# liayan/Legion-1

Measured on AMD Instinct MI355X. Metric: sampled edges/s + feature GB/s, 3-hop GraphSAGE ogbn-papers100M at 1/2/4/8 GPU, higher is better.
Workload: dtype int32 ids / f32 rows (verbatim copy)

## Files before the change

legion-1_amd/csrc/internal.h:

```cpp
#pragma once
#include <hip/hip_runtime.h>
#include <cstdint>
#include <cstdio>
#include <cstdlib>
#include <iostream>
#include <string>
#include <vector>

#include "../../include/legion_amd.h"
#include "audit.h"

namespace legion {

void report_error(const char* file, int line, const char* msg, bool hip_failure);
bool error_pending();
bool error_is_fatal();
int64_t ipc_max_bytes();
bool ipc_size_ok(int64_t bytes, const char* who);
bool ipc_export_ok(const void* ptr, const char* who);
int64_t shard_chunk_bytes();
inline void check(hipError_t e, const char* file, int line)
{
    if (e != hipSuccess) report_error(file, line, hipGetErrorString(e), true);
}
#define HIP_CHECK(expr) ::legion::check((expr), __FILE__, __LINE__)
#define HIP_CHECK_LAST() ::legion::check(hipGetLastError(), __FILE__, __LINE__)
#define LEGION_ARG_ERROR(msg) ::legion::report_error(__FILE__, __LINE__, (msg), false)

std::ostream& log_out();
FILE* log_file();

int physical_device(int logical);
bool is_remote_device(int logical);
struct DeviceGuard {
    int prev = -1, prev_logical = -1;
    explicit DeviceGuard(int logical);
    ~DeviceGuard();
};

int chunk_shift(int64_t unit_bytes, int min_shift);
inline int chunk_count(int64_t n, int shift) { return n > 0 ? (int)(((n - 1) >> shift) + 1) : 1; }
template <typename T>
struct ChunkList {
    std::vector<T*> chunks;
    bool imported = false;
    T* at(int q) const { return q >= 0 && q < (int)chunks.size() ? chunks[q] : nullptr; }
    bool complete(size_t n) const { for (T* p : chunks) if (!p) return false; return chunks.size() == n; }
    void release();
    int export_chunk(int dev, int q, void* handle64, const char* who) const;
    int import_chunk(int q, const void* handle64, int64_t floor_bytes, int open_dev, const char* who);
};
template <typename T> void upload_table(int viewer, const std::vector<T*>& h, T**& tab, bool realloc, const char* what);

typedef unsigned long long pos_t;
constexpr int kPosShift = 32;
constexpr uint32_t kProvisional = 0x80000000u, kPosValueMask = 0x7FFFFFFFu;
constexpr uint32_t kEpochTop = 0xFFFFFFFFu, kSerialLimit = 0xFFFFFFF0u;
__host__ __device__ inline pos_t pos_entry(uint32_t epoch, uint32_t value) { return ((pos_t)epoch << kPosShift) | (pos_t)value; }
#ifndef LEGION_KTILE
#define LEGION_KTILE 1024
#endif
constexpr int kTile = LEGION_KTILE;
constexpr int kBlock = 256;
static_assert(kTile >= kBlock && kTile <= 2048 && (kTile & (kTile - 1)) == 0, "LEGION_KTILE: a power of two in [256, 2048] (k_sample stages 16 bytes of row descriptor per slot in static LDS)");
constexpr int kMaxChunks = 2048;
static_assert(kMaxChunks % kBlock == 0 && kMaxChunks >= 256 * 8, "kMaxChunks: a multiple of the workgroup size, >= 256 CUs x 8 workgroups");
constexpr int ilog2_c(int v) { return v <= 1 ? 0 : 1 + ilog2_c(v >> 1); }
constexpr int kMaxParts = LEGION_MAX_DEVICE;

constexpr int kModes = 3;
static_assert(LEGION_TRAINMODE == 0 && LEGION_VALIDMODE == 1 && LEGION_TESTMODE == 2, "seed sets are indexed by mode");
struct BuildInfoSeedFields {
    const int32_t* LegionBuildInfo::*num;
    const int32_t* const* LegionBuildInfo::*ids;
    const int32_t* const* LegionBuildInfo::*labels;
};
constexpr BuildInfoSeedFields kBuildInfoSeeds[kModes] = {
    {&LegionBuildInfo::training_set_num, &LegionBuildInfo::training_set_ids, &LegionBuildInfo::training_labels},
    {&LegionBuildInfo::validation_set_num, &LegionBuildInfo::validation_set_ids, &LegionBuildInfo::validation_labels},
    {&LegionBuildInfo::testing_set_num, &LegionBuildInfo::testing_set_ids, &LegionBuildInfo::testing_labels}};

constexpr uint32_t kP31 = 2147483647u;
constexpr uint32_t kA = 48271u;

__host__ __device__ inline uint32_t mulmod31(uint32_t a, uint32_t b)
{
    uint64_t p = (uint64_t)a * (uint64_t)b;
    uint32_t r = (uint32_t)(p & kP31) + (uint32_t)(p >> 31);
    r = (r & kP31) + (r >> 31);
    return r >= kP31 ? r - kP31 : r;
}

__host__ __device__ inline uint32_t powmod31(uint32_t base, uint64_t e)
{
    uint32_t r = 1;
    while (e) {
        if (e & 1) r = mulmod31(r, base);
        base = mulmod31(base, base);
        e >>= 1;
    }
    return r;
}

struct FastDiv {
    uint32_t d = 1, m = 0, s = 0;
    FastDiv() = default;
    explicit FastDiv(uint32_t div);
};

struct CsrTables {
    const int64_t* indptr;
    const int32_t* indices;
    const int64_t* const* frag_indptr;
    const int32_t* const* frag_indices;
    int32_t ip_nch, ix_nch, row_shift, edge_shift;
    int32_t partition_count;
    const int8_t* topo_owner;
// ... 223 lines not shown
```

legion-1_amd/csrc/kernels.hip:

```cpp
#include "internal.h"
#include <hipcub/hipcub.hpp>
#include <mutex>
#include <cstring>

#include "audit_hooks.h"

namespace legion {

__device__ inline int32_t sample_index(uint32_t x, int32_t deg)
{
    double result = (double)(uint32_t)(x - 1u);
    result /= 2147483646.0;
    return (int32_t)(result * (double)deg + 0.0);
}

__device__ inline uint32_t fdiv(uint32_t n, const FastDiv& d)
{
    return d.d == 1 ? n : (uint32_t)(((uint64_t)n * d.m) >> d.s);
}

__device__ inline int lane_id() { return threadIdx.x & 63; }
__device__ inline int wave_id() { return threadIdx.x >> 6; }

__device__ inline int32_t total_nodes(const int32_t* nc, int32_t hops) { return nc[5 + 2 * hops]; }
// ... 45 lines not shown
    const int64_t n_init = min((int64_t)max(size, 0) * f_next, (int64_t)aux_cap);
    for (int64_t i = idx; i < n_init; i += (int64_t)gridDim.x * blockDim.x) aux_next[i] = -1;
}
__global__ void k_fill_aux(const int32_t* __restrict__ nc, int32_t count, int32_t* __restrict__ aux, int32_t aux_cap)
{
    const int64_t n = min((int64_t)nc[2] * count, (int64_t)aux_cap);
    for (int64_t i = threadIdx.x + (int64_t)blockDim.x * blockIdx.x; i < n; i += (int64_t)gridDim.x * blockDim.x) aux[i] = -1;
}
__global__ void k_set_cursor(BatchCtl* ctl, int32_t counter, uint32_t epoch) { ctl->counter = counter; ctl->epoch = epoch; }
__global__ void k_advance(BatchCtl* ctl) { ctl->counter += 1; ctl->epoch -= 1; }


struct SampleArgs {
    CsrTables csr;
    const int32_t* sampled_ids;
    const int32_t* agg_src_ids;
    const int32_t* nc;
    const int32_t* ec;
    pos_t* pos_map;
    int32_t* cand;
    int32_t* aux;
    int32_t* tile_edge;
    unsigned long long* edge_access_time;
    const BatchCtl* ctl;
    const uint32_t* pow_tab;
    uint32_t a_tile;
    uint32_t a_step;
    FastDiv fdiv;
    int32_t count;
    int32_t op_id;
    int32_t window;
    int32_t prefilter_from_op;
};

__device__ inline int32_t claim_slot(const SampleArgs& a, uint32_t epoch, int32_t dst, int32_t idx)
{
    const pos_t prov0 = pos_entry(epoch, kProvisional);
    const pos_t mine = prov0 | (pos_t)(uint32_t)idx;
    pos_t cur = (a.op_id < a.prefilter_from_op) ? ~(pos_t)0 : a.pos_map[dst];
    if (cur > mine) {
        const pos_t old = atomicMin(a.pos_map + dst, mine);
        if (old > mine) {
            if ((uint32_t)(old >> kPosShift) == epoch) a.aux[(uint32_t)old & kPosValueMask] = -2 - idx;
            cur = mine;
        } else {
            cur = old;
        }
    }
    if (cur < prov0) return (int32_t)((uint32_t)cur & kPosValueMask);
    if (cur < mine) return -2 - (int32_t)((uint32_t)cur & kPosValueMask);
    return -1;
}

template <bool PRESC, bool PARTITIONED>
__global__ __launch_bounds__(kBlock) void k_sample(SampleArgs a)
{
    __shared__ const int32_t* s_row[kTile + 2];
    __shared__ int32_t s_deg[kTile + 2];
    __shared__ int32_t s_src[kTile + 2];
    __shared__ int32_t s_cnt[kBlock / 64];

    const int32_t N = a.nc[2];
    const int32_t f = a.count;
    const int32_t total = N * f;
    const int32_t* __restrict__ input = (a.op_id == 2) ? a.sampled_ids : a.agg_src_ids + a.ec[2];
    const int32_t n_tiles = (total + kTile - 1) / kTile;
    const int tid = threadIdx.x;
    const uint32_t epoch = a.ctl->epoch;

    if ((int32_t)blockIdx.x >= n_tiles) return;

    uint32_t x[kTile / kBlock];
    {
        uint32_t base = powmod31(a.a_tile, (uint64_t)blockIdx.x);
#pragma unroll
        for (int s = 0; s < kTile / kBlock; s++) x[s] = mulmod31(base, a.pow_tab[tid + kBlock * s]);
    }

    for (int32_t tile = blockIdx.x; tile < n_tiles; tile += gridDim.x) {
        const int32_t tile_start = tile * kTile;
        const int32_t tile_end = min(tile_start + kTile, total);
        const int32_t i0 = (int32_t)fdiv((uint32_t)tile_start, a.fdiv);
        const int32_t i_last = (int32_t)fdiv((uint32_t)(tile_end - 1), a.fdiv);
        const int32_t nrows = i_last - i0 + 1;

        for (int32_t r = tid; r < nrows; r += kBlock) {
            const int32_t src = input[i0 + r];
            const int32_t* rowp = nullptr;
            int32_t deg = -1;
            if (src >= 0) {
                const int64_t* ip = a.csr.indptr + src;
                const int32_t* ix = a.csr.indices;
                int8_t owner = -1;
                if (PARTITIONED && !PRESC) owner = a.csr.topo_owner[src];
                if (owner >= 0) {
                    const int32_t row = a.csr.topo_row[src];
                    ip = a.csr.frag_indptr[owner * a.csr.ip_nch + (row >> a.csr.row_shift)] + (row & ((1 << a.csr.row_shift) - 1));
                    const int64_t start = ip[0];
                    ix = a.csr.frag_indices[owner * a.csr.ix_nch + (int32_t)(start >> a.csr.edge_shift)];
                    rowp = ix + (start & ((1ll << a.csr.edge_shift) - 1));
                    deg = (int32_t)(ip[1] - start);
                } else {
                    const int64_t start = ip[0];
                    rowp = ix + start;
                    deg = (int32_t)(ip[1] - start);
                }
            }
            s_row[r] = rowp;
            s_deg[r] = deg;
            s_src[r] = src;
        }
        __syncthreads();

        int32_t cnt = 0;
#pragma unroll
        for (int s = 0; s < kTile / kBlock; s++) {
            const int32_t idx = tile_start + tid + kBlock * s;
            int32_t dst = -1, known = -1, j = 0, r = 0;
            if (idx < tile_end) {
                const uint32_t i = fdiv((uint32_t)idx, a.fdiv);
                j = idx - (int32_t)i * f;
                r = (int32_t)i - i0;
                const int32_t deg = s_deg[r];
                if (j < deg) {
                    dst = s_row[r][sample_index(x[s], deg)];
                    if (dst < 0) dst = -1;
                }
            }
            int32_t dup = 0;
            for (int d = 1; d <= a.window; d++) {
                const int32_t o = __shfl_up(dst, d);
                if (d <= j && d <= lane_id() && o == dst) dup = d;
            }
            if (dst >= 0) {
                if (PRESC) atomicAdd(a.edge_access_time + s_src[r], 1ull);
                if (dup) known = -2 - (idx - dup);
                else known = claim_slot(a, epoch, dst, idx);
                cnt++;
            }
            if (idx < tile_end) {
                a.cand[idx] = dst;
                if (dst < 0) a.aux[idx] = 0;
                else if (known != -1) a.aux[idx] = known;
            }
        }
        for (int o = 32; o > 0; o >>= 1) cnt += __shfl_down(cnt, o);
        if (lane_id() == 0) s_cnt[wave_id()] = cnt;
        __syncthreads();
        if (tid == 0) {
            int32_t t = 0;
#pragma unroll
            for (int w = 0; w < kBlock / 64; w++) t += s_cnt[w];
            a.tile_edge[tile] = t;
        }
#pragma unroll
        for (int s = 0; s < kTile / kBlock; s++) x[s] = mulmod31(x[s], a.a_step);
        __syncthreads();
    }
}

constexpr int32_t kWinBase = 0x40000000;

__device__ inline int32_t enc_win(int32_t r) { return -2 - (kWinBase + r); }
__device__ inline bool is_win(int32_t v) { return v <= -2 - kWinBase; }
__device__ inline int32_t win_rank(int32_t v) { return -2 - v - kWinBase; }

__host__ __device__ inline FastDiv make_fastdiv(uint32_t div)
{
    FastDiv f;
    f.d = div ? div : 1;
    if (f.d == 1) { f.m = 0; f.s = 0; return f; }
    uint32_t l = 0;
    while ((1ull << l) < f.d) l++;
    f.m = (uint32_t)(((1ull << (31 + l)) / f.d) + 1ull);
    f.s = 31 + l;
    return f;
}

__global__ __launch_bounds__(kBlock) void k_mark(const int32_t* __restrict__ nc, const int32_t* __restrict__ ec,
                                                 int32_t count, int32_t* __restrict__ aux, const int32_t* __restrict__ tile_edge,
                                                 int32_t* __restrict__ tile_node, int2* __restrict__ tile_pre,
                                                 int2* __restrict__ chunk_tot, HopState* __restrict__ hs)
{
    constexpr int S = kTile / kBlock, W = kBlock / 64;
    __shared__ int32_t s_c[S * W];
    const int32_t total = nc[2] * count;
    const int32_t n_tiles = (total + kTile - 1) / kTile;
    const int lane = lane_id(), wave = wave_id();
    const unsigned long long lt = (1ull << lane) - 1ull;
    if (blockIdx.x == 0 && threadIdx.x == 0) {
        HopState h;
        h.edge_base = ec[0]; h.node_base = nc[0]; h.n_edges = 0; h.n_nodes = 0;
        h.in_off = ec[2]; h.n_in = nc[2]; h.slots = total; h.pad = 0;
        *hs = h;
    }
    const int32_t T = (n_tiles + (int32_t)gridDim.x - 1) / (int32_t)gridDim.x;
    const int32_t t0 = (int32_t)blockIdx.x * T, t1 = min(t0 + T, n_tiles);
    if (t0 >= n_tiles) return;
    int32_t nxt[S];
#pragma unroll
    for (int s = 0; s < S; s++) {
        const int64_t idx = (int64_t)t0 * kTile + threadIdx.x + kBlock * s;
        nxt[s] = idx < total ? aux[idx] : 0;
    }
    int32_t te_next = threadIdx.x == 0 ? tile_edge[t0] : 0, run_e = 0, run_n = 0;
    for (int32_t tile = t0; tile < t1; tile++) {
        bool win[S];
        int32_t rk[S];
        const int32_t te = te_next;
#pragma unroll
        for (int s = 0; s < S; s++) {
            const int32_t idx = tile * kTile + threadIdx.x + kBlock * s;
            win[s] = idx < total && nxt[s] == -1;
        }
        {
            const int64_t nt = (int64_t)tile + 1;
#pragma unroll
            for (int s = 0; s < S; s++) {
                const int64_t idx = nt * kTile + threadIdx.x + kBlock * s;
                nxt[s] = (nt < t1 && idx < total) ? aux[idx] : 0;
            }
            if (threadIdx.x == 0 && nt < t1) te_next = tile_edge[nt];
        }
#pragma unroll
        for (int s = 0; s < S; s++) {
            const unsigned long long b = __ballot(win[s]);
            rk[s] = __popcll(b & lt);
            if (lane == 0) s_c[s * W + wave] = __popcll(b);
        }
        __syncthreads();
        int32_t run = 0, before[S];
#pragma unroll
        for (int q = 0; q < S * W; q++) {
#pragma unroll
            for (int s = 0; s < S; s++)
                if (q == s * W + wave) before[s] = run;
            run += s_c[q];
        }
#pragma unroll
        for (int s = 0; s < S; s++)
            if (win[s]) aux[tile * kTile + threadIdx.x + kBlock * s] = enc_win(before[s] + rk[s]);
        if (threadIdx.x == 0) {
            tile_node[tile] = run;
            tile_pre[tile] = make_int2(run_e, run_n);
            run_e += te; run_n += run;
        }
        __syncthreads();
    }
    if (threadIdx.x == 0) chunk_tot[blockIdx.x] = make_int2(run_e, run_n);
}

__device__ inline void apply_update_counter(int32_t* nc, int32_t* ec, int32_t op_id, int32_t hops, int32_t n_nodes,
                                            int32_t n_edges)
{
    const int32_t hh = op_id / 2;
    nc[0] += n_nodes;
    nc[3 + 2 * hh] = nc[1 + 2 * hh] + nc[2 + 2 * hh];
    nc[4 + 2 * hh] = n_nodes;
    if (hh == hops) nc[5 + 2 * hh] = nc[3 + 2 * hh] + nc[4 + 2 * hh];
    nc[1] = 0;
    nc[2] = n_edges;
    ec[2 + hh] = (hh == 1 ? ec[3] : ec[1 + hh]) + n_edges;
    ec[2] = ec[0];
    ec[0] += n_edges;
    ec[1] = 0;
}

struct WriteArgs {
    HopState* hs;
    int32_t* nc;
    int32_t* ec;
    int32_t hops;
    const int32_t* cand;
    const int32_t* aux;
    const int32_t* tile_edge;
    const int32_t* tile_node;
    int32_t* sampled_ids;
    int32_t* agg_src_ids;
    int32_t* agg_src_off;
    int32_t* agg_dst_off;
    pos_t* pos_map;
    FastDiv fdiv;
    int32_t op_id;
    const BatchCtl* ctl;
    int32_t last_hop;
    const int2* tile_pre;
    const int2* chunk_tot;
    int32_t mark_grid;
    int32_t* aux_next;
    int32_t next_count;
    int32_t aux_cap;
    int32_t ids_cap;
    int32_t V;
};

#define LEGION_STORE_OK(i, cap) ((uint32_t)(i) < (uint32_t)(cap))

__global__ __launch_bounds__(kBlock) void k_write(WriteArgs a)
{
    constexpr int S = kTile / kBlock, W = kBlock / 64;
    __shared__ int2 s_chunk[kMaxChunks];
    __shared__ int32_t s_e[S * W];
    __shared__ int2 s_scan[W];
    __shared__ uint32_t s_div_t[3];
    const HopState h = *a.hs;
    const uint32_t epoch = a.ctl->epoch;
    const int32_t total = h.slots;
    const int32_t n_tiles = (total + kTile - 1) / kTile;
    const int lane = lane_id(), wave = wave_id();
    const unsigned long long lt = (1ull << lane) - 1ull;
    if (n_tiles == 0) {
        if (blockIdx.x == 0 && threadIdx.x == 0) apply_update_counter(a.nc, a.ec, a.op_id, a.hops, 0, 0);
        return;
    }
    if ((int32_t)blockIdx.x >= n_tiles) return;
    const int32_t T = (n_tiles + a.mark_grid - 1) / a.mark_grid;
    if (threadIdx.x == 0) {
        const FastDiv f = make_fastdiv((uint32_t)T);
        s_div_t[0] = f.d; s_div_t[1] = f.m; s_div_t[2] = f.s;
    }
    const int32_t n_chunks = (n_tiles + T - 1) / T;
    {
        constexpr int PER = kMaxChunks / kBlock;
        const int32_t q0 = (int32_t)threadIdx.x * PER;
        int2 v[PER];
#pragma unroll
        for (int u = 0; u < PER; u++) v[u] = a.chunk_tot[min(q0 + u, n_chunks - 1)];
        int32_t se = 0, sn = 0;
#pragma unroll
        for (int u = 0; u < PER; u++) {
            if (q0 + u >= n_chunks) v[u] = make_int2(0, 0);
            se += v[u].x; sn += v[u].y;
        }
        int32_t ie = se, in = sn;
        for (int o = 1; o < 64; o <<= 1) {
            const int32_t ue = __shfl_up(ie, o), un = __shfl_up(in, o);
            if (lane >= o) { ie += ue; in += un; }
        }
        if (lane == 63) s_scan[wave] = make_int2(ie, in);
        __syncthreads();
        int32_t run_e = ie - se, run_n = in - sn;
#pragma unroll
        for (int w = 0; w < W; w++)
            if (w < wave) { run_e += s_scan[w].x; run_n += s_scan[w].y; }
#pragma unroll
        for (int u = 0; u < PER; u++) {
            if (q0 + u < n_chunks) s_chunk[q0 + u] = make_int2(run_e, run_n);
            run_e += v[u].x; run_n += v[u].y;
        }
        __syncthreads();
    }
    FastDiv div_t;
    div_t.d = s_div_t[0]; div_t.m = s_div_t[1]; div_t.s = s_div_t[2];
    auto nodes_before = [&](int32_t t, int32_t pre_n_in_chunk) { return s_chunk[fdiv((uint32_t)t, div_t)].y + pre_n_in_chunk; };

    for (int32_t tile = blockIdx.x; tile < n_tiles; tile += gridDim.x) {
        const int2 own = a.tile_pre[tile], own_chunk = s_chunk[fdiv((uint32_t)tile, div_t)];
        const int32_t pre_e = own_chunk.x + own.x, pre_n = own_chunk.y + own.y;
        const int32_t tile_e = a.tile_edge[tile];
        const int32_t ebase = h.edge_base + pre_e;
        const int32_t nbase = h.node_base + pre_n;
        int32_t c[S], so[S], dpos[S], w[S], re[S], wpre[S];
        const int32_t* __restrict__ pre_n_of = reinterpret_cast<const int32_t*>(a.tile_pre) + 1;
#pragma unroll
        for (int s = 0; s < S; s++) {
            const int32_t idx = tile * kTile + threadIdx.x + kBlock * s;
            c[s] = (idx < total) ? a.cand[idx] : -1;
            so[s] = (idx < total) ? a.aux[idx] : 0;
        }
#pragma unroll
        for (int s = 0; s < S; s++) {
            dpos[s] = 0; w[s] = -1;
            if (c[s] == -1) continue;
            const int32_t idx = tile * kTile + threadIdx.x + kBlock * s;
            const int32_t i = (int32_t)fdiv((uint32_t)idx, a.fdiv);
            dpos[s] = (a.op_id == 2) ? (int32_t)((uint32_t)a.pos_map[a.sampled_ids[i]] & kPosValueMask) : a.agg_src_off[h.in_off + i];
            wpre[s] = 0;
            if (so[s] < -1 && !is_win(so[s])) { w[s] = -2 - so[s]; so[s] = a.aux[w[s]]; wpre[s] = pre_n_of[2 * (w[s] / kTile)]; }
        }
#pragma unroll
        for (int s = 0; s < S; s++)
            while (w[s] >= 0 && so[s] < -1 && !is_win(so[s])) { w[s] = -2 - so[s]; so[s] = a.aux[w[s]]; wpre[s] = pre_n_of[2 * (w[s] / kTile)]; }
#pragma unroll
        for (int s = 0; s < S; s++) {
            const unsigned long long be = __ballot(c[s] != -1);
            re[s] = __popcll(be & lt);
            if (lane == 0) s_e[s * W + wave] = __popcll(be);
        }
        __syncthreads();
        if (tile == n_tiles - 1 && threadIdx.x == 0) {
            const int32_t n_edges = pre_e + tile_e, n_nodes = pre_n + a.tile_node[tile];
            a.hs->n_edges = n_edges;
            a.hs->n_nodes = n_nodes;
            apply_update_counter(a.nc, a.ec, a.op_id, a.hops, n_nodes, n_edges);
        }
#pragma unroll
        for (int s = 0; s < S; s++) {
            if (c[s] == -1) continue;
            int32_t pe = 0;
            for (int q = 0; q < s * W + wave; q++) pe += s_e[q];
            const int32_t dst = c[s];
            const int32_t e = ebase + pe + re[s];
            if (!LEGION_STORE_OK(e, a.ids_cap)) continue;
            if (!a.last_hop) a.agg_src_ids[e] = dst;
            a.agg_dst_off[e] = dpos[s];
            int32_t p = so[s];
            if (w[s] >= 0) {
                if (p < -1)
                    p = h.node_base + nodes_before(w[s] / kTile, wpre[s]) + win_rank(p);
            } else if (is_win(p)) {
                p = nbase + win_rank(p);
                if (LEGION_STORE_OK(p, a.ids_cap)) a.sampled_ids[p] = dst;
                if (!a.last_hop && LEGION_STORE_OK(dst, a.V)) a.pos_map[dst] = pos_entry(epoch, (uint32_t)p);
            }
            a.agg_src_off[e] = p;
        }
        if (a.next_count > 0) {
            const int64_t lo = min((int64_t)pre_e * a.next_count, (int64_t)a.aux_cap);
            const int64_t hi = min((int64_t)(pre_e + tile_e) * a.next_count, (int64_t)a.aux_cap);
            for (int64_t q = lo + threadIdx.x; q < hi; q += kBlock) a.aux_next[q] = -1;
        }
        __syncthreads();
    }
}

__global__ __launch_bounds__(kBlock) void k_find_feat(const int32_t* __restrict__ sampled_ids,
                                                      int32_t* __restrict__ cache_offset,
                                                      const int32_t* __restrict__ nc, int32_t off_idx,
                                                      int32_t size_idx, const int32_t* __restrict__ feat_map)
{
    const int32_t off = nc[off_idx], n = nc[size_idx];
    for (int32_t r = threadIdx.x + blockDim.x * blockIdx.x; r < n; r += gridDim.x * blockDim.x) {
        int32_t id = sampled_ids[off + r];
        cache_offset[r] = (id < 0 || !feat_map) ? -1 : feat_map[id];
    }
}

__global__ __launch_bounds__(kBlock) void k_find_topo(const int32_t* __restrict__ input_ids,
                                                      int8_t* __restrict__ part_index,
                                                      int32_t* __restrict__ part_offset, int32_t n,
                                                      const int8_t* __restrict__ owner,
                                                      const int32_t* __restrict__ row)
{
    for (int32_t i = threadIdx.x + blockDim.x * blockIdx.x; i < n; i += gridDim.x * blockDim.x) {
        int32_t id = input_ids[i];
        bool ok = id >= 0 && owner;
        part_index[i] = ok ? owner[id] : (int8_t)-1;
        part_offset[i] = ok ? row[id] : -1;
    }
}

struct GatherKArgs {
    GatherArgs g;
    FastDiv div_c;
    FastDiv div_cap;
};

typedef float v4f __attribute__((ext_vector_type(4)));

__global__ __launch_bounds__(kBlock) void k_row_ptrs(GatherKArgs a)
{
    constexpr int U = 4;
// ... 389 lines not shown
}
static inline int grid_for(int64_t work_items, int per_block, int blocks_per_cu = 8)
{
    int64_t need = (work_items + per_block - 1) / per_block;
    int64_t cap = (int64_t)cu_count() * blocks_per_cu;
    if (need < 1) need = 1;
    return (int)(need < cap ? need : cap);
}

static uint32_t* pow_table()
{
    static uint32_t* tabs[64] = {nullptr};
    static std::mutex mu;
    std::lock_guard<std::mutex> lk(mu);
    int dev = 0;
    HIP_CHECK(hipGetDevice(&dev));
    if (!tabs[dev]) {
        std::vector<uint32_t> h(kTile);
        uint32_t x = 1;
        for (int m = 0; m < kTile; m++) { x = mulmod31(x, kA); h[m] = x; }
        HIP_CHECK(hipMalloc(&tabs[dev], kTile * sizeof(uint32_t)));
        HIP_CHECK(hipMemcpy(tabs[dev], h.data(), kTile * sizeof(uint32_t), hipMemcpyHostToDevice));
    }
    LEGION_AUDIT_SHARE(tabs[dev], current_logical_device());
    return tabs[dev];
}

void launch_seed(hipStream_t s, int32_t* batch_ids, int32_t* labels, int32_t batch_size, int32_t size, int32_t counter,
                 const int32_t* all_ids, const int32_t* all_labels, int32_t total_cap, pos_t* pos_map,
                 uint32_t epoch, BatchCtl* ctl, bool self_driven, int32_t* nc, int32_t* ec, int32_t* aux_next,
                 int32_t f_next, int32_t aux_cap)
{
    const int32_t bound = self_driven ? batch_size : size;
    int blocks = bound > 0 ? (bound - 1) / kBlock + 1 : 1;
    LEGION_AUDIT_LAUNCH(s, "k_seed", LEGION_AW(batch_ids), LEGION_AW(labels), LEGION_AW(pos_map), LEGION_AW(ctl), LEGION_AW(nc), LEGION_AW(ec), LEGION_AW(aux_next), LEGION_AL(all_ids), LEGION_AL(all_labels));
    if (self_driven) k_seed<true><<<blocks, kBlock, 0, s>>>(batch_ids, labels, batch_size, size, counter, all_ids, all_labels, total_cap, pos_map, epoch, ctl, nc, ec, aux_next, f_next, aux_cap);
    else k_seed<false><<<blocks, kBlock, 0, s>>>(batch_ids, labels, batch_size, size, counter, all_ids, all_labels, total_cap, pos_map, epoch, ctl, nc, ec, aux_next, f_next, aux_cap);
    HIP_CHECK_LAST();
}
void launch_set_cursor(hipStream_t s, BatchCtl* ctl, int32_t counter, uint32_t epoch)
{
    LEGION_AUDIT_LAUNCH(s, "k_set_cursor", LEGION_AW(ctl));
    k_set_cursor<<<1, 1, 0, s>>>(ctl, counter, epoch);
    HIP_CHECK_LAST();
}
void launch_advance(hipStream_t s, BatchCtl* ctl)
{
    LEGION_AUDIT_LAUNCH(s, "k_advance", LEGION_AW(ctl));
    k_advance<<<1, 1, 0, s>>>(ctl);
    HIP_CHECK_LAST();
}
void warm_static_tables() { (void)pow_table(); (void)cu_count(); }

void launch_sample_hop(hipStream_t s, const CsrTables& csr, const SamplerBuffers& b, int32_t count, int32_t op_id,
                       int32_t hops, int32_t slots_bound, bool is_presc)
{
    if (count <= 0 || slots_bound <= 0) { LEGION_ARG_ERROR("GPU_Random_Sampling: empty hop"); return; }
    const int max_tiles = (slots_bound + kTile - 1) / kTile;
    constexpr int wg_per_cu = 4;
    const int grid = std::min(grid_for(max_tiles, 1, wg_per_cu), kMaxChunks);
    if (!b.aux_prepared) {
        LEGION_AUDIT_LAUNCH(s, "k_fill_aux", LEGION_AW(b.aux), LEGION_AL(b.nc));
        k_fill_aux<<<grid_for(slots_bound, kBlock * 4), kBlock, 0, s>>>(b.nc, count, b.aux, b.aux_cap);
        HIP_CHECK_LAST();
    }
    SampleArgs a;
    a.csr = csr;
    a.sampled_ids = b.sampled_ids; a.agg_src_ids = b.agg_src_ids; a.nc = b.nc; a.ec = b.ec;
    a.pos_map = b.pos_map; a.cand = b.cand; a.aux = b.aux; a.tile_edge = b.tile_edge;
    a.edge_access_time = b.edge_access_time;
    a.ctl = b.ctl;
    a.pow_tab = pow_table();
    a.a_tile = powmod31(kA, kTile);
    a.a_step = powmod31(kA, (uint64_t)kTile * (uint64_t)grid);
    a.fdiv = FastDiv((uint32_t)count);
    a.count = count; a.op_id = op_id;
    a.window = std::min(count - 1, 8);
    a.prefilter_from_op = 4;
    const bool part = csr.topo_owner != nullptr;
    LEGION_AUDIT_LAUNCH(s, "k_sample", LEGION_AW(a.pos_map), LEGION_AW(a.cand), LEGION_AW(a.aux), LEGION_AW(a.tile_edge), LEGION_AW(a.edge_access_time), LEGION_AL(a.sampled_ids), LEGION_AL(a.agg_src_ids), LEGION_AL(a.nc), LEGION_AL(a.ec), LEGION_AL(a.ctl), LEGION_AL(a.pow_tab), LEGION_AL(csr.frag_indptr), LEGION_AL(csr.frag_indices), LEGION_AL(csr.topo_owner), LEGION_AL(csr.topo_row), LEGION_AR(csr.indptr), LEGION_AR(csr.indices));
    if (is_presc) k_sample<true, false><<<grid, kBlock, 0, s>>>(a);
    else if (part) k_sample<false, true><<<grid, kBlock, 0, s>>>(a);
    else k_sample<false, false><<<grid, kBlock, 0, s>>>(a);
    HIP_CHECK_LAST();
    LEGION_AUDIT_LAUNCH(s, "k_mark", LEGION_AW(b.aux), LEGION_AW(b.tile_node), LEGION_AW(b.tile_pre), LEGION_AW(b.chunk_tot), LEGION_AW(b.hop_state), LEGION_AL(b.nc), LEGION_AL(b.ec), LEGION_AL(b.tile_edge));
    k_mark<<<grid, kBlock, 0, s>>>(b.nc, b.ec, count, b.aux, b.tile_edge, b.tile_node, b.tile_pre, b.chunk_tot, b.hop_state);
    HIP_CHECK_LAST();
    WriteArgs w;
    w.hs = b.hop_state; w.nc = b.nc; w.ec = b.ec; w.hops = hops; w.cand = b.cand; w.aux = b.aux; w.ctl = b.ctl; w.tile_edge = b.tile_edge; w.tile_node = b.tile_node;
    w.sampled_ids = b.sampled_ids; w.agg_src_ids = b.agg_src_ids; w.agg_src_off = b.agg_src_off;
    w.agg_dst_off = b.agg_dst_off; w.pos_map = b.pos_map; w.fdiv = a.fdiv; w.op_id = op_id; w.last_hop = (op_id / 2 == hops) ? 1 : 0;
    w.aux_next = b.aux_next; w.next_count = b.next_count; w.aux_cap = b.aux_cap; w.ids_cap = b.ids_cap; w.V = b.V;
    w.tile_pre = b.tile_pre; w.chunk_tot = b.chunk_tot; w.mark_grid = grid;
    const int wgrid = grid_for(max_tiles, 1, 8);
    LEGION_AUDIT_LAUNCH(s, "k_write", LEGION_AW(w.hs), LEGION_AW(w.nc), LEGION_AW(w.ec), LEGION_AW(w.sampled_ids), LEGION_AW(w.agg_src_ids), LEGION_AW(w.agg_src_off), LEGION_AW(w.agg_dst_off), LEGION_AW(w.pos_map), LEGION_AW(w.aux_next), LEGION_AL(w.cand), LEGION_AL(w.aux), LEGION_AL(w.tile_edge), LEGION_AL(w.tile_node), LEGION_AL(w.tile_pre), LEGION_AL(w.chunk_tot), LEGION_AL(w.ctl));
    k_write<<<wgrid, kBlock, 0, s>>>(w);
    HIP_CHECK_LAST();
}

void launch_find_feat(hipStream_t s, const int32_t* sampled_ids, int32_t* cache_offset, const int32_t* nc,
                      int32_t op_id, const int32_t* feat_map, int32_t bound)
{
    const int l = (op_id - 1) / 2;
    LEGION_AUDIT_LAUNCH(s, "k_find_feat", LEGION_AW(cache_offset), LEGION_AL(sampled_ids), LEGION_AL(nc), LEGION_AL(feat_map));
    k_find_feat<<<grid_for(bound, kBlock), kBlock, 0, s>>>(sampled_ids, cache_offset, nc, 3 + 2 * l, 4 + 2 * l, feat_map);
    HIP_CHECK_LAST();
}

void launch_find_topo(hipStream_t s, const int32_t* input_ids, int8_t* part_index, int32_t* part_offset,
                      int32_t batch_size, const int8_t* topo_owner, const int32_t* topo_row)
{
    if (batch_size <= 0) return;
    LEGION_AUDIT_LAUNCH(s, "k_find_topo", LEGION_AW(part_index), LEGION_AW(part_offset), LEGION_AL(input_ids), LEGION_AL(topo_owner), LEGION_AL(topo_row));
    k_find_topo<<<grid_for(batch_size, kBlock), kBlock, 0, s>>>(input_ids, part_index, part_offset, batch_size, topo_owner, topo_row);
    HIP_CHECK_LAST();
}

void launch_gather(hipStream_t s, const GatherArgs& g, int32_t rows_bound)
{
    if (g.F <= 0 || rows_bound <= 0) return;
    GatherKArgs a;
    a.g = g;
    a.div_cap = FastDiv((uint32_t)(g.cache_capacity > 0 ? g.cache_capacity : 1));
    LEGION_AUDIT_LAUNCH(s, "k_gather", LEGION_AW(g.dst), LEGION_AW(g.row_ptr), LEGION_AW(g.rows_seen), LEGION_AW(g.hit_stats), LEGION_AL(g.sampled_ids), LEGION_AL(g.nc), LEGION_AL(g.feat_map), LEGION_AL(g.shard_tab), LEGION_AR(g.table));
    bool vec4 = (g.F % 4 == 0) && (((uintptr_t)g.table | (uintptr_t)g.dst) % 16 == 0);
    const int C = vec4 ? g.F / 4 : g.F;
    const int lanes = C;
    if ((int64_t)rows_bound * lanes >= (1ll << 31)) { LEGION_ARG_ERROR("get_feature_kernel: rows*F exceeds 2^31 work items"); return; }
    a.div_c = FastDiv((uint32_t)C);
    int grid;
    bool fused = false;
    if (g.row_ptr && !g.row_ptr_ready) {
        fused = !g.hit_stats && !g.table_on_host;
        if (!fused) {
            const int64_t est_rows = g.rows_hint > 0 ? std::min<int64_t>(rows_bound, (int64_t)g.rows_hint + g.rows_hint / 4 + 1024) : rows_bound;
            k_row_ptrs<<<grid_for(est_rows, kBlock * 4, 64), kBlock, 0, s>>>(a);
            HIP_CHECK_LAST();
        }
    }
    if (g.rows_hint > 0) {
        const int64_t est = std::min<int64_t>(rows_bound, (int64_t)g.rows_hint + g.rows_hint / 4 + 1024);
        grid = grid_for(est * lanes, kBlock * (g.table_on_host ? 1 : 3), 8192);
    } else {
        grid = grid_for((int64_t)rows_bound * lanes, kBlock, 512);
    }
    if (fused) { if (vec4) k_gather_lookup<v4f, 2><<<grid, kBlock, 0, s>>>(a); else k_gather_lookup<float, 2><<<grid, kBlock, 0, s>>>(a); }
    else if (vec4) k_gather<v4f, 1, 2><<<grid, kBlock, 0, s>>>(a);
    else k_gather<float, 1, 2><<<grid, kBlock, 0, s>>>(a);
    HIP_CHECK_LAST();
}
// ... 192 lines not shown
```

legion-1_amd/csrc/storage.cpp:

```cpp
#include "internal.h"

#include <algorithm>
#include <cstring>
#include <set>

#include "audit_hooks.h"

using namespace legion;

static void enable_p2p(int32_t partition_count)
{
    std::set<int> phys;
    for (int i = 0; i < partition_count; i++) phys.insert(physical_device(i));
    if (audit::on()) for (int a = 0; a < partition_count; a++) for (int b = 0; b < partition_count; b++) if (a != b) audit::record_peer(a, b);
    if (phys.size() < 2) return;
    int cur = 0;
    HIP_CHECK(hipGetDevice(&cur));
    for (int a : phys) {
        HIP_CHECK(hipSetDevice(a));
        for (int b : phys) {
            if (a == b) continue;
            int ok = 0;
            HIP_CHECK(hipDeviceCanAccessPeer(&ok, a, b));
            if (ok) {
// ... 371 lines not shown
int32_t* GPUNodeStorage_GetTrainingLabels(const GPUNodeStorage* n, int32_t p) { return n->seed_set(LEGION_TRAINMODE, p).labels; }
int32_t* GPUNodeStorage_GetValidationLabels(const GPUNodeStorage* n, int32_t p) { return n->seed_set(LEGION_VALIDMODE, p).labels; }
int32_t* GPUNodeStorage_GetTestingLabels(const GPUNodeStorage* n, int32_t p) { return n->seed_set(LEGION_TESTMODE, p).labels; }
int32_t GPUNodeStorage_TrainingSetSize(const GPUNodeStorage* n, int32_t p) { return n->seed_set(LEGION_TRAINMODE, p).num; }
int32_t GPUNodeStorage_ValidationSetSize(const GPUNodeStorage* n, int32_t p) { return n->seed_set(LEGION_VALIDMODE, p).num; }
int32_t GPUNodeStorage_TestingSetSize(const GPUNodeStorage* n, int32_t p) { return n->seed_set(LEGION_TESTMODE, p).num; }
int32_t GPUNodeStorage_TotalNodeNum(const GPUNodeStorage* n) { return n->total_num_nodes; }
float* GPUNodeStorage_GetAllFloatAttr(const GPUNodeStorage* n) { return n->float_attrs; }
int32_t GPUNodeStorage_GetFloatAttrLen(const GPUNodeStorage* n) { return n->float_attr_len; }
void GPUNodeStorage_Delete(GPUNodeStorage* n)
{
    if (!n) return;
    GPUNodeStorage_Finalize(n);
    delete n;
}

}

GPUMemoryPool::GPUMemoryPool(int32_t depth)
{
    pipeline_depth = depth > 0 ? depth : 1;
    float_features.assign(pipeline_depth, nullptr);
    labels.assign(pipeline_depth, nullptr);
    node_counter.assign(pipeline_depth, nullptr);
    edge_counter.assign(pipeline_depth, nullptr);
    sampled_ids.assign(pipeline_depth, nullptr);
    agg_src_off.assign(pipeline_depth, nullptr);
    agg_dst_off.assign(pipeline_depth, nullptr);
}

extern "C" {

GPUMemoryPool* NewGPUMemoryPool(int32_t pipeline_depth) { return new GPUMemoryPool(pipeline_depth); }

void GPUMemoryPool_AllocateScratch(GPUMemoryPool* p, int32_t total_num_nodes, int32_t batch_size,
                                   const int32_t* fanout, int32_t hops)
{
    if (!p || hops < 1 || hops > LEGION_MAX_HOPS || batch_size < 1 || total_num_nodes < 1) { LEGION_ARG_ERROR("GPUMemoryPool_AllocateScratch: bad arguments"); return; }
    if (p->owns_scratch) GPUMemoryPool_Finalize(p);
    p->V = total_num_nodes; p->batch_size = batch_size; p->hops = hops;
    int64_t ids = batch_size, cur = batch_size, max_slots = 0;
    p->level_bound[0] = batch_size;
    for (int h = 0; h < hops; h++) {
        p->fanout[h] = fanout[h];
        cur *= fanout[h];
        if (cur > max_slots) max_slots = cur;
        ids += cur;
        if (ids >= (1ll << 31)) { LEGION_ARG_ERROR("GPUMemoryPool_AllocateScratch: batch*fanouts exceeds int32"); return; }
        if (cur >= (1ll << 30)) { LEGION_ARG_ERROR("GPUMemoryPool_AllocateScratch: a hop of 2^30 or more slots exceeds the slot-state encoding"); return; }
        p->level_bound[h + 1] = (int32_t)cur;
    }
    p->num_ids = (int32_t)ids;
    p->max_slots = (int32_t)max_slots;
    p->max_tiles = (int32_t)((max_slots + kTile - 1) / kTile);
    p->owns_scratch = true;
    HIP_CHECK(hipMalloc(&p->pos_map, (size_t)total_num_nodes * sizeof(pos_t)));
    HIP_CHECK(hipMemset(p->pos_map, 0xFF, (size_t)total_num_nodes * sizeof(pos_t)));
    p->batch_serial = 0;
    HIP_CHECK(hipMalloc(&p->ctl, sizeof(BatchCtl)));
    { const BatchCtl c{0, kEpochTop}; HIP_CHECK(hipMemcpy(p->ctl, &c, sizeof(c), hipMemcpyHostToDevice)); }
    p->ctl_synced = false;
    HIP_CHECK(hipHostMalloc((void**)&p->rows_seen, (LEGION_MAX_HOPS + 2) * sizeof(int32_t), hipHostMallocMapped));
    memset(p->rows_seen, 0, (LEGION_MAX_HOPS + 2) * sizeof(int32_t));
    HIP_CHECK(hipHostGetDevicePointer((void**)&p->rows_seen_dev, p->rows_seen, 0));
    HIP_CHECK(hipMalloc(&p->cand, (size_t)p->max_slots * sizeof(int32_t)));
    for (auto& a : p->aux2) HIP_CHECK(hipMalloc(&a, (size_t)p->max_slots * sizeof(int32_t)));
    HIP_CHECK(hipMalloc(&p->tile_edge, (size_t)(p->max_tiles + 1) * sizeof(int32_t)));
    HIP_CHECK(hipMalloc(&p->tile_node, (size_t)(p->max_tiles + 1) * sizeof(int32_t)));
    HIP_CHECK(hipMalloc(&p->tile_pre, (size_t)(p->max_tiles + 1) * sizeof(int2)));
    HIP_CHECK(hipMalloc(&p->chunk_tot, (size_t)kMaxChunks * sizeof(int2)));
    HIP_CHECK(hipMalloc(&p->hop_state, sizeof(HopState)));
    HIP_CHECK(hipMalloc(&p->cache_search_buffer, (size_t)p->num_ids * sizeof(int32_t)));
    HIP_CHECK(hipMalloc((void**)&p->row_ptr, (size_t)p->num_ids * sizeof(float*)));
    HIP_CHECK(hipMalloc(&p->agg_src_ids, (size_t)p->num_ids * sizeof(int32_t)));
    HIP_CHECK(hipMalloc(&p->tmp_part_ind, (size_t)p->num_ids));
    HIP_CHECK(hipMalloc(&p->tmp_part_off, (size_t)p->num_ids * sizeof(int32_t)));
    HIP_CHECK(hipDeviceSynchronize());
}
int32_t GPUMemoryPool_NumIds(const GPUMemoryPool* p) { return p->num_ids; }

#define POOL_PIPE_SETTER(name, field, type) \
    void GPUMemoryPool_Set##name(GPUMemoryPool* p, type* ptr, int32_t pipe) { \
        if (pipe < 0 || pipe >= p->pipeline_depth) { LEGION_ARG_ERROR("GPUMemoryPool_Set" #name ": bad pipe"); return; } \
        p->field[pipe] = ptr; } \
    type* GPUMemoryPool_Get##name(const GPUMemoryPool* p) { return p->field[p->current_pipe]; }
POOL_PIPE_SETTER(SampledIds, sampled_ids, int32_t)
POOL_PIPE_SETTER(FloatFeatures, float_features, float)
POOL_PIPE_SETTER(Labels, labels, int32_t)
POOL_PIPE_SETTER(AggSrcOf, agg_src_off, int32_t)
POOL_PIPE_SETTER(AggDstOf, agg_dst_off, int32_t)
POOL_PIPE_SETTER(NodeCounter, node_counter, int32_t)
POOL_PIPE_SETTER(EdgeCounter, edge_counter, int32_t)
#undef POOL_PIPE_SETTER
void GPUMemoryPool_SetFeatureRows(GPUMemoryPool* p, int32_t rows) { p->feature_rows = rows; }
void GPUMemoryPool_SetCurrentPipe(GPUMemoryPool* p, int32_t pipe) { p->current_pipe = pipe % p->pipeline_depth; }
void GPUMemoryPool_SetCurrentMode(GPUMemoryPool* p, int32_t mode) { p->mode = mode; }
void GPUMemoryPool_SetIter(GPUMemoryPool* p, int32_t iter) { p->iter = iter; }
int32_t GPUMemoryPool_GetCurrentMode(const GPUMemoryPool* p) { return p->mode; }
int32_t GPUMemoryPool_GetIter(const GPUMemoryPool* p) { return p->iter; }
int32_t* GPUMemoryPool_GetAggSrcId(const GPUMemoryPool* p) { return p->agg_src_ids; }
int32_t* GPUMemoryPool_GetCacheSearchBuffer(const GPUMemoryPool* p) { return p->cache_search_buffer; }
char* GPUMemoryPool_GetTmpPartIdx(const GPUMemoryPool* p) { return (char*)p->tmp_part_ind; }
int32_t* GPUMemoryPool_GetTmpPartOff(const GPUMemoryPool* p) { return p->tmp_part_off; }
uint64_t* GPUMemoryPool_GetPositionMap(const GPUMemoryPool* p) { return (uint64_t*)p->pos_map; }
int32_t* GPUMemoryPool_GetCandidateBuffer(const GPUMemoryPool* p) { return p->cand; }
uint32_t GPUMemoryPool_GetBatchSerial(const GPUMemoryPool* p) { return p->batch_serial; }
void GPUMemoryPool_SetBatchSerial(GPUMemoryPool* p, uint32_t serial) { p->batch_serial = serial; p->ctl_synced = false; }
// ... 21 lines not shown
```

Measured before the change: 6.318 billion.

## Use narrow sampler tiles for small hops and prefetch k_write inputs before scan

Templates the sample/mark/write kernels on tile size and picks a 256-slot tile with more workgroups per CU when a hop's slot bound is small, so early hops spread over more workgroups instead of leaving CUs idle. k_write now loads the chunk totals and its first tile's candidate, aux, tile_pre and tile_edge values before the chunk scan, hiding that latency behind the scan. Scratch tile arrays are sized for the larger of the two tilings. The risk is more tiles and chunk-scan overhead on mid-size hops, and the chunk_tot prefetch now reads all kMaxChunks entries rather than clamping to n_chunks.

Result: faster. 6.441 billion, median of 6 (+1.9%).

```diff
diff --git a/legion-1_amd/csrc/internal.h b/legion-1_amd/csrc/internal.h
--- a/legion-1_amd/csrc/internal.h
+++ b/legion-1_amd/csrc/internal.h
@@ -63,6 +63,19 @@
 constexpr int kTile = LEGION_KTILE;
 constexpr int kBlock = 256;
 static_assert(kTile >= kBlock && kTile <= 2048 && (kTile & (kTile - 1)) == 0, "LEGION_KTILE: a power of two in [256, 2048] (k_sample stages 16 bytes of row descriptor per slot in static LDS)");
+#ifndef LEGION_NARROW_SLOTS
+#define LEGION_NARROW_SLOTS (256 * 1024)
+#endif
+constexpr int kTileNarrow = kBlock;
+constexpr int64_t kNarrowSlots = LEGION_NARROW_SLOTS;
+static_assert(kTileNarrow <= kTile, "one pow_tab of kTile entries serves both tile sizes");
+constexpr int64_t sampler_tile_of(int64_t slots_bound) { return slots_bound <= kNarrowSlots ? kTileNarrow : kTile; }
+constexpr int64_t sampler_max_tiles(int64_t max_slots)
+{
+    const int64_t wide = (max_slots + kTile - 1) / kTile, narrow_slots = max_slots < kNarrowSlots ? max_slots : kNarrowSlots;
+    const int64_t narrow = (narrow_slots + kTileNarrow - 1) / kTileNarrow;
+    return wide > narrow ? wide : narrow;
+}
 constexpr int kMaxChunks = 2048;
 static_assert(kMaxChunks % kBlock == 0 && kMaxChunks >= 256 * 8, "kMaxChunks: a multiple of the workgroup size, >= 256 CUs x 8 workgroups");
 constexpr int ilog2_c(int v) { return v <= 1 ? 0 : 1 + ilog2_c(v >> 1); }
diff --git a/legion-1_amd/csrc/kernels.hip b/legion-1_amd/csrc/kernels.hip
--- a/legion-1_amd/csrc/kernels.hip
+++ b/legion-1_amd/csrc/kernels.hip
@@ -121,34 +121,34 @@
     return -1;
 }
 
-template <bool PRESC, bool PARTITIONED>
+template <int TILE, bool PRESC, bool PARTITIONED>
 __global__ __launch_bounds__(kBlock) void k_sample(SampleArgs a)
 {
-    __shared__ const int32_t* s_row[kTile + 2];
-    __shared__ int32_t s_deg[kTile + 2];
-    __shared__ int32_t s_src[kTile + 2];
+    __shared__ const int32_t* s_row[TILE + 2];
+    __shared__ int32_t s_deg[TILE + 2];
+    __shared__ int32_t s_src[TILE + 2];
     __shared__ int32_t s_cnt[kBlock / 64];
 
     const int32_t N = a.nc[2];
     const int32_t f = a.count;
     const int32_t total = N * f;
     const int32_t* __restrict__ input = (a.op_id == 2) ? a.sampled_ids : a.agg_src_ids + a.ec[2];
-    const int32_t n_tiles = (total + kTile - 1) / kTile;
+    const int32_t n_tiles = (total + TILE - 1) / TILE;
     const int tid = threadIdx.x;
     const uint32_t epoch = a.ctl->epoch;
 
     if ((int32_t)blockIdx.x >= n_tiles) return;
 
-    uint32_t x[kTile / kBlock];
+    uint32_t x[TILE / kBlock];
     {
         uint32_t base = powmod31(a.a_tile, (uint64_t)blockIdx.x);
 #pragma unroll
-        for (int s = 0; s < kTile / kBlock; s++) x[s] = mulmod31(base, a.pow_tab[tid + kBlock * s]);
+        for (int s = 0; s < TILE / kBlock; s++) x[s] = mulmod31(base, a.pow_tab[tid + kBlock * s]);
     }
 
     for (int32_t tile = blockIdx.x; tile < n_tiles; tile += gridDim.x) {
-        const int32_t tile_start = tile * kTile;
-        const int32_t tile_end = min(tile_start + kTile, total);
+        const int32_t tile_start = tile * TILE;
+        const int32_t tile_end = min(tile_start + TILE, total);
         const int32_t i0 = (int32_t)fdiv((uint32_t)tile_start, a.fdiv);
         const int32_t i_last = (int32_t)fdiv((uint32_t)(tile_end - 1), a.fdiv);
         const int32_t nrows = i_last - i0 + 1;
@@ -183,7 +183,7 @@
 
         int32_t cnt = 0;
 #pragma unroll
-        for (int s = 0; s < kTile / kBlock; s++) {
+        for (int s = 0; s < TILE / kBlock; s++) {
             const int32_t idx = tile_start + tid + kBlock * s;
             int32_t dst = -1, known = -1, j = 0, r = 0;
             if (idx < tile_end) {
@@ -223,7 +223,7 @@
             a.tile_edge[tile] = t;
         }
 #pragma unroll
-        for (int s = 0; s < kTile / kBlock; s++) x[s] = mulmod31(x[s], a.a_step);
+        for (int s = 0; s < TILE / kBlock; s++) x[s] = mulmod31(x[s], a.a_step);
         __syncthreads();
     }
 }
@@ -246,15 +246,16 @@
     return f;
 }
 
+template <int TILE>
 __global__ __launch_bounds__(kBlock) void k_mark(const int32_t* __restrict__ nc, const int32_t* __restrict__ ec,
                                                  int32_t count, int32_t* __restrict__ aux, const int32_t* __restrict__ tile_edge,
                                                  int32_t* __restrict__ tile_node, int2* __restrict__ tile_pre,
                                                  int2* __restrict__ chunk_tot, HopState* __restrict__ hs)
 {
-    constexpr int S = kTile / kBlock, W = kBlock / 64;
+    constexpr int S = TILE / kBlock, W = kBlock / 64;
     __shared__ int32_t s_c[S * W];
     const int32_t total = nc[2] * count;
-    const int32_t n_tiles = (total + kTile - 1) / kTile;
+    const int32_t n_tiles = (total + TILE - 1) / TILE;
     const int lane = lane_id(), wave = wave_id();
     const unsigned long long lt = (1ull << lane) - 1ull;
     if (blockIdx.x == 0 && threadIdx.x == 0) {
@@ -269,7 +270,7 @@
     int32_t nxt[S];
 #pragma unroll
     for (int s = 0; s < S; s++) {
-        const int64_t idx = (int64_t)t0 * kTile + threadIdx.x + kBlock * s;
+        const int64_t idx = (int64_t)t0 * TILE + threadIdx.x + kBlock * s;
         nxt[s] = idx < total ? aux[idx] : 0;
     }
     int32_t te_next = threadIdx.x == 0 ? tile_edge[t0] : 0, run_e = 0, run_n = 0;
@@ -279,14 +280,14 @@
         const int32_t te = te_next;
 #pragma unroll
         for (int s = 0; s < S; s++) {
-            const int32_t idx = tile * kTile + threadIdx.x + kBlock * s;
+            const int32_t idx = tile * TILE + threadIdx.x + kBlock * s;
             win[s] = idx < total && nxt[s] == -1;
         }
         {
             const int64_t nt = (int64_t)tile + 1;
 #pragma unroll
             for (int s = 0; s < S; s++) {
-                const int64_t idx = nt * kTile + threadIdx.x + kBlock * s;
+                const int64_t idx = nt * TILE + threadIdx.x + kBlock * s;
                 nxt[s] = (nt < t1 && idx < total) ? aux[idx] : 0;
             }
             if (threadIdx.x == 0 && nt < t1) te_next = tile_edge[nt];
@@ -308,7 +309,7 @@
         }
 #pragma unroll
         for (int s = 0; s < S; s++)
-            if (win[s]) aux[tile * kTile + threadIdx.x + kBlock * s] = enc_win(before[s] + rk[s]);
+            if (win[s]) aux[tile * TILE + threadIdx.x + kBlock * s] = enc_win(before[s] + rk[s]);
         if (threadIdx.x == 0) {
             tile_node[tile] = run;
             tile_pre[tile] = make_int2(run_e, run_n);
@@ -365,17 +366,32 @@
 
 #define LEGION_STORE_OK(i, cap) ((uint32_t)(i) < (uint32_t)(cap))
 
+template <int TILE>
 __global__ __launch_bounds__(kBlock) void k_write(WriteArgs a)
 {
-    constexpr int S = kTile / kBlock, W = kBlock / 64;
+    constexpr int S = TILE / kBlock, W = kBlock / 64;
     __shared__ int2 s_chunk[kMaxChunks];
     __shared__ int32_t s_e[S * W];
     __shared__ int2 s_scan[W];
     __shared__ uint32_t s_div_t[3];
+    constexpr int PER = kMaxChunks / kBlock;
+    const int32_t q0 = (int32_t)threadIdx.x * PER;
+    int2 v[PER];
+#pragma unroll
+    for (int u = 0; u < PER; u++) v[u] = a.chunk_tot[q0 + u];
+    int32_t c[S], so[S];
+#pragma unroll
+    for (int s = 0; s < S; s++) {
+        const int64_t idx = (int64_t)blockIdx.x * TILE + threadIdx.x + kBlock * s;
+        c[s] = idx < a.aux_cap ? a.cand[idx] : -1;
+        so[s] = idx < a.aux_cap ? a.aux[idx] : 0;
+    }
+    int2 own = a.tile_pre[blockIdx.x];
+    int32_t tile_e = a.tile_edge[blockIdx.x];
     const HopState h = *a.hs;
     const uint32_t epoch = a.ctl->epoch;
     const int32_t total = h.slots;
-    const int32_t n_tiles = (total + kTile - 1) / kTile;
+    const int32_t n_tiles = (total + TILE - 1) / TILE;
     const int lane = lane_id(), wave = wave_id();
     const unsigned long long lt = (1ull << lane) - 1ull;
     if (n_tiles == 0) {
@@ -390,11 +406,6 @@
     }
     const int32_t n_chunks = (n_tiles + T - 1) / T;
     {
-        constexpr int PER = kMaxChunks / kBlock;
-        const int32_t q0 = (int32_t)threadIdx.x * PER;
-        int2 v[PER];
-#pragma unroll
-        for (int u = 0; u < PER; u++) v[u] = a.chunk_tot[min(q0 + u, n_chunks - 1)];
         int32_t se = 0, sn = 0;
 #pragma unroll
         for (int u = 0; u < PER; u++) {
@@ -424,32 +435,35 @@
     auto nodes_before = [&](int32_t t, int32_t pre_n_in_chunk) { return s_chunk[fdiv((uint32_t)t, div_t)].y + pre_n_in_chunk; };
 
     for (int32_t tile = blockIdx.x; tile < n_tiles; tile += gridDim.x) {
-        const int2 own = a.tile_pre[tile], own_chunk = s_chunk[fdiv((uint32_t)tile, div_t)];
+        const bool first = tile == (int32_t)blockIdx.x;
+        if (!first) { own = a.tile_pre[tile]; tile_e = a.tile_edge[tile]; }
+        const int2 own_chunk = s_chunk[fdiv((uint32_t)tile, div_t)];
         const int32_t pre_e = own_chunk.x + own.x, pre_n = own_chunk.y + own.y;
-        const int32_t tile_e = a.tile_edge[tile];
         const int32_t ebase = h.edge_base + pre_e;
         const int32_t nbase = h.node_base + pre_n;
-        int32_t c[S], so[S], dpos[S], w[S], re[S], wpre[S];
+        int32_t dpos[S], w[S], re[S], wpre[S];
         const int32_t* __restrict__ pre_n_of = reinterpret_cast<const int32_t*>(a.tile_pre) + 1;
 #pragma unroll
         for (int s = 0; s < S; s++) {
-            const int32_t idx = tile * kTile + threadIdx.x + kBlock * s;
-            c[s] = (idx < total) ? a.cand[idx] : -1;
-            so[s] = (idx < total) ? a.aux[idx] : 0;
+            const int32_t idx = tile * TILE + threadIdx.x + kBlock * s;
+            if (!first) {
+                c[s] = (idx < total) ? a.cand[idx] : -1;
+                so[s] = (idx < total) ? a.aux[idx] : 0;
+            } else if (idx >= total) { c[s] = -1; so[s] = 0; }
         }
 #pragma unroll
         for (int s = 0; s < S; s++) {
             dpos[s] = 0; w[s] = -1;
             if (c[s] == -1) continue;
-            const int32_t idx = tile * kTile + threadIdx.x + kBlock * s;
+            const int32_t idx = tile * TILE + threadIdx.x + kBlock * s;
             const int32_t i = (int32_t)fdiv((uint32_t)idx, a.fdiv);
             dpos[s] = (a.op_id == 2) ? (int32_t)((uint32_t)a.pos_map[a.sampled_ids[i]] & kPosValueMask) : a.agg_src_off[h.in_off + i];
             wpre[s] = 0;
-            if (so[s] < -1 && !is_win(so[s])) { w[s] = -2 - so[s]; so[s] = a.aux[w[s]]; wpre[s] = pre_n_of[2 * (w[s] / kTile)]; }
+            if (so[s] < -1 && !is_win(so[s])) { w[s] = -2 - so[s]; so[s] = a.aux[w[s]]; wpre[s] = pre_n_of[2 * (w[s] / TILE)]; }
         }
 #pragma unroll
         for (int s = 0; s < S; s++)
-            while (w[s] >= 0 && so[s] < -1 && !is_win(so[s])) { w[s] = -2 - so[s]; so[s] = a.aux[w[s]]; wpre[s] = pre_n_of[2 * (w[s] / kTile)]; }
+            while (w[s] >= 0 && so[s] < -1 && !is_win(so[s])) { w[s] = -2 - so[s]; so[s] = a.aux[w[s]]; wpre[s] = pre_n_of[2 * (w[s] / TILE)]; }
 #pragma unroll
         for (int s = 0; s < S; s++) {
             const unsigned long long be = __ballot(c[s] != -1);
@@ -476,7 +490,7 @@
             int32_t p = so[s];
             if (w[s] >= 0) {
                 if (p < -1)
-                    p = h.node_base + nodes_before(w[s] / kTile, wpre[s]) + win_rank(p);
+                    p = h.node_base + nodes_before(w[s] / TILE, wpre[s]) + win_rank(p);
             } else if (is_win(p)) {
                 p = nbase + win_rank(p);
                 if (LEGION_STORE_OK(p, a.ids_cap)) a.sampled_ids[p] = dst;
@@ -972,12 +986,12 @@
 }
 void warm_static_tables() { (void)pow_table(); (void)cu_count(); }
 
-void launch_sample_hop(hipStream_t s, const CsrTables& csr, const SamplerBuffers& b, int32_t count, int32_t op_id,
+template <int TILE>
+static void launch_sample_hop_t(hipStream_t s, const CsrTables& csr, const SamplerBuffers& b, int32_t count, int32_t op_id,
                        int32_t hops, int32_t slots_bound, bool is_presc)
 {
-    if (count <= 0 || slots_bound <= 0) { LEGION_ARG_ERROR("GPU_Random_Sampling: empty hop"); return; }
-    const int max_tiles = (slots_bound + kTile - 1) / kTile;
-    constexpr int wg_per_cu = 4;
+    const int max_tiles = (slots_bound + TILE - 1) / TILE;
+    constexpr int wg_per_cu = TILE == kTile ? 4 : 8;
     const int grid = std::min(grid_for(max_tiles, 1, wg_per_cu), kMaxChunks);
     if (!b.aux_prepared) {
         LEGION_AUDIT_LAUNCH(s, "k_fill_aux", LEGION_AW(b.aux), LEGION_AL(b.nc));
@@ -991,20 +1005,20 @@
     a.edge_access_time = b.edge_access_time;
     a.ctl = b.ctl;
     a.pow_tab = pow_table();
-    a.a_tile = powmod31(kA, kTile);
-    a.a_step = powmod31(kA, (uint64_t)kTile * (uint64_t)grid);
+    a.a_tile = powmod31(kA, TILE);
+    a.a_step = powmod31(kA, (uint64_t)TILE * (uint64_t)grid);
     a.fdiv = FastDiv((uint32_t)count);
     a.count = count; a.op_id = op_id;
     a.window = std::min(count - 1, 8);
     a.prefilter_from_op = 4;
     const bool part = csr.topo_owner != nullptr;
     LEGION_AUDIT_LAUNCH(s, "k_sample", LEGION_AW(a.pos_map), LEGION_AW(a.cand), LEGION_AW(a.aux), LEGION_AW(a.tile_edge), LEGION_AW(a.edge_access_time), LEGION_AL(a.sampled_ids), LEGION_AL(a.agg_src_ids), LEGION_AL(a.nc), LEGION_AL(a.ec), LEGION_AL(a.ctl), LEGION_AL(a.pow_tab), LEGION_AL(csr.frag_indptr), LEGION_AL(csr.frag_indices), LEGION_AL(csr.topo_owner), LEGION_AL(csr.topo_row), LEGION_AR(csr.indptr), LEGION_AR(csr.indices));
-    if (is_presc) k_sample<true, false><<<grid, kBlock, 0, s>>>(a);
-    else if (part) k_sample<false, true><<<grid, kBlock, 0, s>>>(a);
-    else k_sample<false, false><<<grid, kBlock, 0, s>>>(a);
+    if (is_presc) k_sample<TILE, true, false><<<grid, kBlock, 0, s>>>(a);
+    else if (part) k_sample<TILE, false, true><<<grid, kBlock, 0, s>>>(a);
+    else k_sample<TILE, false, false><<<grid, kBlock, 0, s>>>(a);
     HIP_CHECK_LAST();
     LEGION_AUDIT_LAUNCH(s, "k_mark", LEGION_AW(b.aux), LEGION_AW(b.tile_node), LEGION_AW(b.tile_pre), LEGION_AW(b.chunk_tot), LEGION_AW(b.hop_state), LEGION_AL(b.nc), LEGION_AL(b.ec), LEGION_AL(b.tile_edge));
-    k_mark<<<grid, kBlock, 0, s>>>(b.nc, b.ec, count, b.aux, b.tile_edge, b.tile_node, b.tile_pre, b.chunk_tot, b.hop_state);
+    k_mark<TILE><<<grid, kBlock, 0, s>>>(b.nc, b.ec, count, b.aux, b.tile_edge, b.tile_node, b.tile_pre, b.chunk_tot, b.hop_state);
     HIP_CHECK_LAST();
     WriteArgs w;
     w.hs = b.hop_state; w.nc = b.nc; w.ec = b.ec; w.hops = hops; w.cand = b.cand; w.aux = b.aux; w.ctl = b.ctl; w.tile_edge = b.tile_edge; w.tile_node = b.tile_node;
@@ -1014,8 +1028,16 @@
     w.tile_pre = b.tile_pre; w.chunk_tot = b.chunk_tot; w.mark_grid = grid;
     const int wgrid = grid_for(max_tiles, 1, 8);
     LEGION_AUDIT_LAUNCH(s, "k_write", LEGION_AW(w.hs), LEGION_AW(w.nc), LEGION_AW(w.ec), LEGION_AW(w.sampled_ids), LEGION_AW(w.agg_src_ids), LEGION_AW(w.agg_src_off), LEGION_AW(w.agg_dst_off), LEGION_AW(w.pos_map), LEGION_AW(w.aux_next), LEGION_AL(w.cand), LEGION_AL(w.aux), LEGION_AL(w.tile_edge), LEGION_AL(w.tile_node), LEGION_AL(w.tile_pre), LEGION_AL(w.chunk_tot), LEGION_AL(w.ctl));
-    k_write<<<wgrid, kBlock, 0, s>>>(w);
-    HIP_CHECK_LAST();
+    k_write<TILE><<<wgrid, kBlock, 0, s>>>(w);
+    HIP_CHECK_LAST();
+}
+
+void launch_sample_hop(hipStream_t s, const CsrTables& csr, const SamplerBuffers& b, int32_t count, int32_t op_id,
+                       int32_t hops, int32_t slots_bound, bool is_presc)
+{
+    if (count <= 0 || slots_bound <= 0) { LEGION_ARG_ERROR("GPU_Random_Sampling: empty hop"); return; }
+    if (sampler_tile_of(slots_bound) == kTileNarrow) launch_sample_hop_t<kTileNarrow>(s, csr, b, count, op_id, hops, slots_bound, is_presc);
+    else launch_sample_hop_t<kTile>(s, csr, b, count, op_id, hops, slots_bound, is_presc);
 }
 
 void launch_find_feat(hipStream_t s, const int32_t* sampled_ids, int32_t* cache_offset, const int32_t* nc,
diff --git a/legion-1_amd/csrc/storage.cpp b/legion-1_amd/csrc/storage.cpp
--- a/legion-1_amd/csrc/storage.cpp
+++ b/legion-1_amd/csrc/storage.cpp
@@ -447,7 +447,7 @@
     }
     p->num_ids = (int32_t)ids;
     p->max_slots = (int32_t)max_slots;
-    p->max_tiles = (int32_t)((max_slots + kTile - 1) / kTile);
+    p->max_tiles = (int32_t)sampler_max_tiles(max_slots);
     p->owns_scratch = true;
     HIP_CHECK(hipMalloc(&p->pos_map, (size_t)total_num_nodes * sizeof(pos_t)));
     HIP_CHECK(hipMemset(p->pos_map, 0xFF, (size_t)total_num_nodes * sizeof(pos_t)));
```
